# lijiaman/egoego_release

Hardware: AMD Instinct MI355X
Metric: diffusion-steps/sec (B=256, T=120, 22-joint) (higher is better)
Workload: dtype i8x3 + bf16x3 (attention layer, fc, FFN and linear_out: 2 x int8 slices per operand, int32 accumulate; embed: split-bf16, fp32 accumulate)

## Files before the change

### egoego_release_amd/csrc/egoego_hip.hip

```cpp
#include "../../include/egoego_hip.h"

#include <math.h>
#include <stdarg.h>
#include <stdio.h>
#include <stdlib.h>
#include <string.h>

#include <string>
#include <vector>

#include "attention.h"
#include "attn_layer_i8.h"
#include "attn_layer_i8w.h"
#include "attn_layer_i8h.h"
#include "attn_split_i8.h"
#include "attn_core_i8.h"
#include "attn_core_i8w.h"
#include "common.h"
#include "gemm.h"
#include "pointwise.h"
#include "tail_fused.h"

template __global__ void qkv_i8_kernel<EpiQK<2>, EpiV<2>>(QkvI8Args, EpiQK<2>, EpiV<2>);

// ... 403 lines not shown
        once.done();
    }
    if (rows / 64 >= 256) {
        c->last_kernel[EGOEGO_K_FC_LN] = FFN8 ? "tail_kernel<2,true,false>" : "tail_kernel<2,false,false>";
        tail_kernel<2, FFN8, false><<<dim3(rows / 64), dim3(256), tail_smem_bytes(2), s>>>(ta);
    } else if (!FFN8 && TAIL8_BF16 && rows / 32 <= TAIL8_BF16_MAX_BLOCKS) {
        c->last_kernel[EGOEGO_K_FC_LN] = "tail_kernel<1,false,false,false,8>";
        tail_kernel<1, false, false, false, 8><<<dim3(rows / 32), dim3(512), tail_smem_bytes(1, 8), s>>>(ta);
    } else {
        c->last_kernel[EGOEGO_K_FC_LN] = FFN8 ? "tail_kernel<1,true,false>" : "tail_kernel<1,false,false>";
        tail_kernel<1, FFN8, false><<<dim3(rows / 32), dim3(256), tail_smem_bytes(1), s>>>(ta);
    }
    HIP_TRY(hipGetLastError());
    return 0;
}
#ifndef ATTN_SPLIT_MAX_BLOCKS
#define ATTN_SPLIT_MAX_BLOCKS 256
#endif
#ifndef ATTN_SPLIT6_MAX_BLOCKS
#define ATTN_SPLIT6_MAX_BLOCKS 256
#endif
#ifndef ATTN_SPLIT2_MAX_BLOCKS
#define ATTN_SPLIT2_MAX_BLOCKS 192
#endif
#ifndef ATTN_HALF_MAX_BLOCKS
#define ATTN_HALF_MAX_BLOCKS 192
#endif
#ifndef EMBED8_MAX_BLOCKS
#define EMBED8_MAX_BLOCKS 256
#endif
#ifndef TAIL8_MAX_BLOCKS
#define TAIL8_MAX_BLOCKS 256
#endif
static int launch_tail(egoego_ctx* c, const TailArgs& ta, int rows, hipStream_t s, bool resident = false) {
    if (ta.fc8) {
        static DevOnce once;
        if (once.pending()) {
            HIP_TRY(allow_smem((tail_kernel<1, true, true, true>), tail_smem_bytes(1) + TAIL_PAR_BYTES));
            HIP_TRY(allow_smem((tail_kernel<1, true, true, false, 8>), tail_smem_bytes(1, 8) + TAIL_PAR_BYTES));
            HIP_TRY(allow_smem((tail_kernel<1, true, true, true, 4, true>), tail_smem_bytes(1) + TAIL_PAR_BYTES + TAIL_RES_BYTES));
            HIP_TRY(allow_smem((tail_kernel<1, true, true, false, 8, true>), tail_smem_bytes(1, 8) + TAIL_PAR_BYTES + TAIL_RES_BYTES));
            once.done();
        }
        if (resident) {
            if (rows / 32 > TAIL8_MAX_BLOCKS) {
                c->last_kernel[EGOEGO_K_FC_LN] = "tail_kernel<1,true,true,true,4,true>";
                tail_kernel<1, true, true, true, 4, true><<<dim3(rows / 32), dim3(256), tail_smem_bytes(1) + TAIL_PAR_BYTES + TAIL_RES_BYTES, s>>>(ta);
            } else {
                c->last_kernel[EGOEGO_K_FC_LN] = "tail_kernel<1,true,true,false,8,true>";
                tail_kernel<1, true, true, false, 8, true><<<dim3(rows / 32), dim3(512), tail_smem_bytes(1, 8) + TAIL_PAR_BYTES + TAIL_RES_BYTES, s>>>(ta);
            }
            HIP_TRY(hipGetLastError());
            return 0;
        }
        if (rows / 32 > TAIL8_MAX_BLOCKS) {
            c->last_kernel[EGOEGO_K_FC_LN] = "tail_kernel<1,true,true,true>";
            tail_kernel<1, true, true, true><<<dim3(rows / 32), dim3(256), tail_smem_bytes(1) + TAIL_PAR_BYTES, s>>>(ta);
        } else {
            c->last_kernel[EGOEGO_K_FC_LN] = "tail_kernel<1,true,true,false,8>";
            tail_kernel<1, true, true, false, 8><<<dim3(rows / 32), dim3(512), tail_smem_bytes(1, 8) + TAIL_PAR_BYTES, s>>>(ta);
        }
        HIP_TRY(hipGetLastError());
        return 0;
    }
    return ta.ffn8 ? launch_tail_f<true>(c, ta, rows, s) : launch_tail_f<false>(c, ta, rows, s);
}


template <int TT>
static int launch_embed_tt(const EmbedArgs& ea, int rows, hipStream_t s) {
    static DevOnce once;
    if (once.pending()) {
        HIP_TRY(allow_smem((embed_kernel<TT, 4>), TT * 32 * 1024));
        HIP_TRY(allow_smem((embed_kernel<TT, 8>), TT * 32 * 1024));
        once.done();
    }
    if (rows / (32 * TT) <= EMBED8_MAX_BLOCKS)
        embed_kernel<TT, 8><<<dim3(rows / (32 * TT)), dim3(512), TT * 32 * 1024, s>>>(ea);
    else
        embed_kernel<TT, 4><<<dim3(rows / (32 * TT)), dim3(256), TT * 32 * 1024, s>>>(ea);
    HIP_TRY(hipGetLastError());
    return 0;
}
template <int TT, bool I8, bool IDS>
static int launch_out_tt(const OutArgsT<IDS>& oa, int rows, hipStream_t s) {
    static DevOnce once;
    if (once.pending()) {
        HIP_TRY(allow_smem((out_kernel<TT, 1, I8, IDS>), TT * 32 * 1024));
        HIP_TRY(allow_smem((out_kernel<TT, 2, I8, IDS>), TT * 32 * 1024));
        once.done();
    }
    const int nb = rows / (32 * TT);
    if (nb <= 128)
// ... 1163 lines not shown
```

### egoego_release_amd/csrc/gemm.h

```cpp
#pragma once
#include <type_traits>

#include "common.h"

#ifndef EGOEGO_ABLATE_MAINLOOP
#define EGOEGO_ABLATE_MAINLOOP 0
#endif
#ifdef EGOEGO_PERFDEBUG
#define EG_DBG(...) __VA_ARGS__
#else
#define EG_DBG(...)
#endif

struct GemmOperands {
    const __bf16* w;
    size_t w_plane;
    const __bf16* a;
    size_t a_plane;
    int K16;
    int nfb;
    int ntb;
    int tblk0;
    EG_DBG(int ablate;
           unsigned long long* trace;)
// ... 690 lines not shown
        }
    }
};

template <int NP, int NWF, int BT>
struct EpiResLN {
    static_assert(NWF == 4 || NWF == 8, "4 waves of 4 feature tiles or 8 waves of 2");
    static EG_D float combine(const float* red, int slot) {
        float q[4];
#pragma unroll
        for (int w = 0; w < 4; ++w) q[w] = NWF == 4 ? red[slot + w * BT] : red[slot + 2 * w * BT] + red[slot + (2 * w + 1) * BT];
        return ((q[0] + q[1]) + q[2]) + q[3];
    }
    const float* bias;
    const __bf16* res;
    size_t res_plane;
    const float* gamma;
    const float* beta;
    const float* row_mask;
    __bf16* out;
    size_t out_plane;
    float eps;
    int8_t* q8;
    size_t q8_plane;
    float* q8_scale;
    const int8_t* res8;
    size_t res8_plane;
    const float* res8_scale;
    char* lds_q8;
    float* lds_scale;
    unsigned* outlier;
    float* outlier_park;
    int outlier_rows;
    template <int FT, int TT, class ResR = NoRows, class KeepR = NoRows>
    __device__ void run(f32x16 (&acc)[FT][TT], int f0, int t0, int lane, int wf, int wt, char* smem, const ResR* rr = nullptr,
                        KeepR* keep = nullptr) const {
        constexpr bool RES_REG = !std::is_same<ResR, NoRows>::value, KEEP = !std::is_same<KeepR, NoRows>::value;
        static_assert((!RES_REG && !KEEP) || TT == 1, "register rows: one token tile");
        static_assert(NWF * FT * 32 == 512 && (FT == 2 || FT == 4), "LayerNorm epilogue needs the whole 512-wide row in the block");
        const int hf = lane >> 5, col = lane & 31;
        float* red1 = (float*)smem;
        float* red2 = red1 + TT * NWF * BT;
        float* red3 = red2 + TT * NWF * BT;
        int slot[TT];
        float mean[TT], rstd[TT], amax[TT];
#pragma unroll
        for (int j = 0; j < TT; ++j) {
            const int m = t0 + j * 32 + col;
            slot[j] = (j * NWF) * BT + (wt * TT + j) * 32 + col;
            float s1 = 0.f, pp[FT / 2];
            if (RES_REG || res8) {
                float rs;
                if constexpr (RES_REG) rs = rr->scale; else rs = res8_scale[m];
#pragma unroll
                for (int i = 0; i < FT; ++i) {
                    float r[16];
                    if constexpr (RES_REG) {
                        dequant16(rr->s1[i], rr->s2[i], rs, r);
                    } else {
                        const size_t idx8 = acc_slot_i8(m, f0 + i * 32, hf, 16);
                        dequant16(*(const u32x4*)(res8 + idx8), *(const u32x4*)(res8 + res8_plane + idx8), rs, r);
                    }
#pragma unroll
                    for (int g = 0; g < 4; ++g) {
                        const float4 b4 = *(const float4*)(bias + f0 + i * 32 + 8 * g + 4 * hf);
                        const float bb[4] = {b4.x, b4.y, b4.z, b4.w};
#pragma unroll
                        for (int c = 0; c < 4; ++c) acc[i][j][4 * g + c] += bb[c] + r[4 * g + c];
                    }
                }
            } else
#pragma unroll
            for (int i = 0; i < FT; ++i)
#pragma unroll
                for (int jj = 0; jj < 2; ++jj) {
                    const int fb = f0 + i * 32 + 16 * jj + 4 * hf;
                    const float4 b0 = *(const float4*)(bias + fb);
                    const float4 b1 = *(const float4*)(bias + fb + 8);
                    const size_t idx = acc_slot(m, f0 + i * 32, jj, hf, 32);
                    float r[8];
                    const u32x4 rh = *(const u32x4*)(res + idx);
                    if (NP == 2) {
                        const u32x4 rl = *(const u32x4*)(res + res_plane + idx);
                        unpack8(rh, rl, r);
                    } else {
                        unpack8_hi(rh, r);
                    }
                    const float bb[8] = {b0.x, b0.y, b0.z, b0.w, b1.x, b1.y, b1.z, b1.w};
#pragma unroll
                    for (int c = 0; c < 8; ++c) acc[i][j][8 * jj + c] += bb[c] + r[c];
                }
#pragma unroll
            for (int i2 = 0; i2 < FT / 2; ++i2) {
                float p = 0.f;
#pragma unroll
                for (int i = 2 * i2; i < 2 * i2 + 2; ++i)
#pragma unroll
                    for (int r = 0; r < 16; ++r) p += acc[i][j][r];
                pp[i2] = p + __shfl_xor(p, 32);
            }
            s1 = pp[0];
            if (FT == 4) s1 += pp[FT / 2 - 1];
            if (hf == 0) red1[slot[j] + wf * BT] = s1;
        }
        __syncthreads();
#pragma unroll
        for (int j = 0; j < TT; ++j) {
            mean[j] = combine(red1, slot[j]) * (1.0f / 512.0f);
            float pp[FT / 2];
#pragma unroll
            for (int i2 = 0; i2 < FT / 2; ++i2) {
                float p = 0.f;
#pragma unroll
                for (int i = 2 * i2; i < 2 * i2 + 2; ++i)
#pragma unroll
                    for (int r = 0; r < 16; ++r) {
                        const float d = acc[i][j][r] - mean[j];
                        p += d * d;
                    }
                pp[i2] = p + __shfl_xor(p, 32);
            }
            float s2 = pp[0];
            if (FT == 4) s2 += pp[FT / 2 - 1];
            if (hf == 0) red2[slot[j] + wf * BT] = s2;
        }
        __syncthreads();
#pragma unroll
        for (int j = 0; j < TT; ++j) {
            const int m = t0 + j * 32 + col;
            const float var = combine(red2, slot[j]);
            rstd[j] = 1.0f / sqrtf(var * (1.0f / 512.0f) + eps);
            const float mk = row_mask ? row_mask[m] : 1.0f;
            amax[j] = 0.f;
#pragma unroll
            for (int i = 0; i < FT; ++i)
#pragma unroll
                for (int jj = 0; jj < 2; ++jj) {
                    const int fb = f0 + i * 32 + 16 * jj + 4 * hf;
                    const float4 g0 = *(const float4*)(gamma + fb), g1 = *(const float4*)(gamma + fb + 8);
                    const float4 e0 = *(const float4*)(beta + fb), e1 = *(const float4*)(beta + fb + 8);
                    const float ga[8] = {g0.x, g0.y, g0.z, g0.w, g1.x, g1.y, g1.z, g1.w};
                    const float be[8] = {e0.x, e0.y, e0.z, e0.w, e1.x, e1.y, e1.z, e1.w};
                    float v[8];
#pragma unroll
                    for (int c = 0; c < 8; ++c) {
                        v[c] = ((acc[i][j][8 * jj + c] - mean[j]) * rstd[j] * ga[c] + be[c]) * mk;
                        acc[i][j][8 * jj + c] = v[c];
                        amax[j] = fmaxf(amax[j], fabsf(v[c]));
                    }
                    if (out) {
                        u32x4 hi, lo;
                        split8(v, hi, lo);
                        const size_t idx = acc_slot(m, f0 + i * 32, jj, hf, 32);
                        *(u32x4*)(out + idx) = hi;
                        if (NP == 2) *(u32x4*)(out + out_plane + idx) = lo;
                    }
                }
            if (q8 || lds_q8) {
                amax[j] = fmaxf(amax[j], __shfl_xor(amax[j], 32));
                if (hf == 0) red3[slot[j] + wf * BT] = amax[j];
            }
        }
        if (q8 || lds_q8) {
            __syncthreads();
#pragma unroll
            for (int j = 0; j < TT; ++j) {
                const int m = t0 + j * 32 + col;
                float rmax = 0.f;
#pragma unroll
                for (int w = 0; w < NWF; ++w) rmax = fmaxf(rmax, red3[slot[j] + w * BT]);
                const float inv = rmax > 0.f ? I8_QMAX / rmax : 0.f;
                const float sc = rmax > 0.f ? rmax / I8_QMAX : 0.f;
                if (wf == 0 && hf == 0) {
                    if (q8_scale) q8_scale[m] = sc;
                    if (lds_scale) lds_scale[(wt * TT + j) * 32 + col] = sc;
                }
                if constexpr (KEEP) keep->scale = sc;
#pragma unroll
                for (int i = 0; i < FT; ++i) {
                    float v[16];
#pragma unroll
                    for (int r = 0; r < 16; ++r) v[r] = acc[i][j][r];
                    u32x4 s1, s2;
                    quant16(v, inv, s1, s2);
                    if (q8) {
                        const size_t idx = acc_slot_i8(m, f0 + i * 32, hf, 16);
                        *(u32x4*)(q8 + idx) = s1;
                        *(u32x4*)(q8 + q8_plane + idx) = s2;
                    }
                    if (lds_q8) {
                        char* d = lds_chunk_slot<TT>(lds_q8, (f0 >> 5) + i, j, lane);
                        *(u32x4*)d = s1;
                        *(u32x4*)(d + TT * 8192) = s2;
                    }
                    if constexpr (KEEP) {
                        keep->s1[i] = s1;
                        keep->s2[i] = s2;
// ... 338 lines not shown
```

### egoego_release_amd/csrc/tail_fused.h

```cpp
#pragma once
#include <type_traits>

#include "gemm.h"

#ifndef TAIL_ABLATE
#define TAIL_ABLATE 0
#endif
#ifndef TAIL_RING1
#define TAIL_RING1 4
#endif
#ifndef TAIL_RING_IO
#define TAIL_RING_IO 4
#endif
#ifndef TAIL8_RING
#define TAIL8_RING 4
#endif
#ifndef TAIL8_RING_FC
#define TAIL8_RING_FC 4
#endif

struct TailArgs {
    const __bf16* o;
    size_t o_plane;
    int HD16;
    const __bf16* wfc;
    size_t wfc_plane;
    EpiResLN<2, 4, 0> ln1;
    const __bf16* w1;
    size_t w1_plane;
    EpiTiled<true, 2> relu;
    const __bf16* w2;
    size_t w2_plane;
    EpiResLN<2, 4, 0> ln2;
    int fc8, H;
    const int8_t* o8;
    size_t o8_plane;
    const float* o_scale;
    const int8_t* wfc8;
    size_t wfc8_plane;
    const float* s_wfc;
    const int8_t* wfc8_3;
    int ffn8;
    const int8_t* w1_8;
    const int8_t* w2_8;
    size_t w8_plane;
    const float* s_w1;
    const float* s_w2;
    EpiReluQ8<4, 0> relu8;
    int stop;
    unsigned* outlier;
    int outlier_rows;
    EG_DBG(unsigned long long* trace;)
};

static constexpr int tail_smem_bytes(int TT, int NWV = 4) { return TT * 32 * 1024 + 3 * TT * NWV * 32 * TT * 4; }
static constexpr int TAIL_PAR_BYTES = 10 * 512 * 4;

using tail_rsrc = __amdgpu_buffer_rsrc_t;
EG_D tail_rsrc tail_make_rsrc(const void* p, size_t bytes) {
    return __builtin_amdgcn_make_buffer_rsrc((void*)p, 0, (int)(bytes < 0x7fffffffu ? bytes : 0x7fffffffu), 0x00020000);
}
EG_D i32x4 tail_load(tail_rsrc r, int voff, unsigned soff) {
    return __builtin_bit_cast(i32x4, __builtin_amdgcn_raw_buffer_load_b128(r, voff, soff, 0));
}

template <int FT, int TT, int RING, bool LAST, int DP, int NKS = 8, bool I8 = false, bool WLO0 = false>
struct TailChunk {
    using AccT = typename std::conditional<I8, I8Acc, f32x16>::type;
    static constexpr int PD = RING - 1, NW = FT * 2;
    static constexpr int NWL = WLO0 ? FT : NW;
    static_assert(!WLO0 || I8, "int8 slices only");
    static_assert(NKS == 8 || (LAST && DP == 0), "only the last chunk may be short");
    static_assert(RING == 2 || RING == 4 || RING == 8, "ring slots must divide the 8 k-steps of a chunk");
    static constexpr int n_ops(int s) { return ((s + PD < NKS || !LAST) ? NWL : 0) + (s == 0 ? DP : 0); }
    static constexpr int after_dma() {
        int n = 0;
        for (int s = 1; s < 8; ++s) n += n_ops(s);
        return n < 63 ? n : 63;
    }
    static constexpr int allowed(int ks) {
        int n = 0;
        if (ks < PD) {
            n += (PD - 1 - ks) * NWL;
            for (int s = 0; s < ks; ++s) n += n_ops(s);
        } else {
            n += ks - PD == 0 ? DP : 0;
            for (int s = ks - PD + 1; s < ks; ++s) n += n_ops(s);
        }
        return n < 63 ? n : 63;
    }
    template <int G>
    static EG_D void mma(i32x4 w, i32x4 a, f32x16& c) {
        if (TAIL_ABLATE & 8) return;
        c = __builtin_amdgcn_mfma_f32_32x32x16_bf16(__builtin_bit_cast(bf16x8, w), __builtin_bit_cast(bf16x8, a), c, 0, 0, 0);
    }
    template <int G>
// ... 66 lines not shown
        }
        step<0>(acc, wq, ah, al, wr, wcur, wnext, act, act_plane, lane, dma);
        if (NKS > 1) step<1>(acc, wq, ah, al, wr, wcur, wnext, act, act_plane, lane, dma);
        if (NKS > 2) step<2>(acc, wq, ah, al, wr, wcur, wnext, act, act_plane, lane, dma);
        if (NKS > 3) step<3>(acc, wq, ah, al, wr, wcur, wnext, act, act_plane, lane, dma);
        if (NKS > 4) step<4>(acc, wq, ah, al, wr, wcur, wnext, act, act_plane, lane, dma);
        if (NKS > 5) step<5>(acc, wq, ah, al, wr, wcur, wnext, act, act_plane, lane, dma);
        if (NKS > 6) step<6>(acc, wq, ah, al, wr, wcur, wnext, act, act_plane, lane, dma);
        if (NKS > 7) step<7>(acc, wq, ah, al, wr, wcur, wnext, act, act_plane, lane, dma);
        if (DP) {
            asm volatile("" ::: "memory");
            wait_counts<after_dma(), 15>();
        }
    }
};

template <int FT, int TT, int RING, bool REM2 = false, bool I8 = false, int NWAVES = 4, bool WLO0 = false>
struct DirectGemm {
    using AccT = typename std::conditional<I8, I8Acc, f32x16>::type;
    static constexpr int NW = 2 * FT, PD = RING - 1;
    static constexpr int CH_PLANE = TT * 8 * 1024, CH_BYTES = 2 * CH_PLANE;
    static constexpr int DMA_PIECES = 16 * TT / NWAVES;
    static constexpr int SMEM_BYTES = 2 * CH_BYTES;

    struct NoPost {
        EG_D void operator()(int) const {}
    };
    struct NoPre {
        EG_D void operator()() const {}
    };
    template <class Mark, class Post = NoPost, class Pre = NoPre>
    static EG_D void run(AccT (&acc)[FT][TT], const __bf16* in, size_t in_plane, int K16, const __bf16* w, size_t w_plane, char* act,
                         int tt0, int wave, int lane, Mark mark, int wtile0 = -1, Post post = Post{}, Pre pre = Pre{}) {
        const int wt0 = wtile0 >= 0 ? wtile0 : wave * FT;
        i32x4 wq[RING][NW];
        const tail_rsrc wr = tail_make_rsrc(w, w_plane * 4);
        const tail_rsrc ir = tail_make_rsrc((const char*)in + (((size_t)tt0 * (size_t)K16) << 10), 0x7fffffffu);
        const unsigned wpb = (unsigned)(w_plane * 2), ipb = (unsigned)(in_plane * 2);
        const int NQ = REM2 ? K16 / 8 + 1 : K16 / 8;
        auto w_offsets = [&](int kb, unsigned (&out)[NW]) {
#pragma unroll
            for (int i = 0; i < FT; ++i)
#pragma unroll
                for (int s = 0; s < 2; ++s) out[2 * i + s] = s * wpb + (unsigned)(((wt0 + i) * K16 + kb) << 10);
        };
        auto dma_piece = [&](int q, int piece) {
            const int x = wave * DMA_PIECES + piece;
            const int s = x / (8 * TT), j = (x >> 3) % TT;
            int kb = x & 7;
            if (REM2 && q == NQ - 1) kb &= 1;
            const unsigned src = s * ipb + (unsigned)((j * K16 + 8 * q + kb) << 10);
            char* dst = act + (q & 1) * CH_BYTES + s * CH_PLANE + ((j * 8 + kb) << 10);
            __builtin_amdgcn_raw_ptr_buffer_load_lds(ir, (__attribute__((address_space(3))) void*)dst, 16, lane * 16, src, 0, 0);
        };
        unsigned wcur[NW], wnext[NW];
#pragma unroll
        for (int pc = 0; pc < DMA_PIECES; ++pc) dma_piece(0, pc);
        w_offsets(0, wcur);
#pragma unroll
        for (int k = 0; k < PD; ++k)
#pragma unroll
            for (int q = 0; q < NW; ++q)
                if (!(WLO0 && (q & 1))) wq[k][q] = tail_load(wr, lane * 16, wcur[q] + (k << 10));
#pragma unroll
        for (int i = 0; i < FT; ++i)
#pragma unroll
            for (int j = 0; j < TT; ++j) acc_zero(acc[i][j]);
        pre();
        asm volatile("s_waitcnt vmcnt(0)" ::: "memory");
        __syncthreads();
        mark();
        for (int q = 0; q + 1 < NQ; ++q) {
            w_offsets(8 * q, wcur);
            w_offsets(8 * q + 8, wnext);
            TailChunk<FT, TT, RING, false, DMA_PIECES, 8, I8, WLO0>::run(acc, wq, wr, wcur, wnext, act + (q & 1) * CH_BYTES, CH_PLANE, lane,
                                                             [&](int piece) { dma_piece(q + 1, piece); });
            post(q);
            __builtin_amdgcn_s_barrier();
            asm volatile("" ::: "memory");
        }
        w_offsets(8 * (NQ - 1), wcur);
        TailChunk<FT, TT, RING, true, 0, (REM2 ? 2 : 8), I8, WLO0>::run(acc, wq, wr, wcur, wcur, act + ((NQ - 1) & 1) * CH_BYTES, CH_PLANE, lane, [](int) {});
        post(NQ - 1);
        __syncthreads();
    }

    static EG_D void prime(i32x4 (&wq)[RING][NW], const __bf16* w, size_t w_plane, int K16, int wt0, int lane) {
        const tail_rsrc wr = tail_make_rsrc(w, w_plane * 4);
        const unsigned wpb = (unsigned)(w_plane * 2);
#pragma unroll
        for (int k = 0; k < PD; ++k)
#pragma unroll
            for (int i = 0; i < FT; ++i)
#pragma unroll
                for (int sl = 0; sl < 2; ++sl) wq[k][2 * i + sl] = tail_load(wr, lane * 16, sl * wpb + (unsigned)(((wt0 + i) * K16 + k) << 10));
    }
    template <class Mark>
    static EG_D void run_resident(AccT (&acc)[FT][TT], i32x4 (&wq)[RING][NW], const __bf16* w, size_t w_plane, const char* act, int lane, Mark mark,
                                  int wt0) {
        static_assert(!REM2, "two whole chunks");
        constexpr int K16 = 16;
        const tail_rsrc wr = tail_make_rsrc(w, w_plane * 4);
        const unsigned wpb = (unsigned)(w_plane * 2);
        auto w_offsets = [&](int kb, unsigned (&out)[NW]) {
#pragma unroll
            for (int i = 0; i < FT; ++i)
#pragma unroll
                for (int sl = 0; sl < 2; ++sl) out[2 * i + sl] = sl * wpb + (unsigned)(((wt0 + i) * K16 + kb) << 10);
        };
        unsigned wcur[NW], wnext[NW];
#pragma unroll
        for (int i = 0; i < FT; ++i)
#pragma unroll
            for (int j = 0; j < TT; ++j) acc_zero(acc[i][j]);
        mark();
        w_offsets(0, wcur);
        w_offsets(8, wnext);
        TailChunk<FT, TT, RING, false, 0, 8, I8>::run(acc, wq, wr, wcur, wnext, act, CH_PLANE, lane, [](int) {});
        TailChunk<FT, TT, RING, true, 0, 8, I8>::run(acc, wq, wr, wnext, wnext, act + CH_BYTES, CH_PLANE, lane, [](int) {});
    }
};

static constexpr int TAIL_RES_BYTES = 272;
template <int TT, bool FFN8, bool FC8 = false, bool W2 = false, int NWV = 4, bool RES = false>
__global__ __launch_bounds__(64 * NWV, ((W2 || NWV == 8) ? 2 : 1)) void tail_kernel(TailArgs a) {
    static_assert(!RES || (FFN8 && FC8 && TT == 1), "LDS-resident FFN operands: the all-int8 32-token tail");
    static_assert(!W2 || (FFN8 && FC8 && TT == 1), "the two-workgroups-per-CU build exists for the all-int8 32-token tail");
    static_assert(NWV == 4 || (NWV == 8 && TT == 1 && !W2 && ((FFN8 && FC8) || (!FFN8 && !FC8 && !RES))),
                  "the eight-wave build exists for the 32-token tails: all int8, or (round 5) all split-bf16");
    constexpr int TOK = 32 * TT, FT = 16 / NWV;
    using G = DirectGemm<FT, TT, 4, false, false, NWV>;
    extern __shared__ __attribute__((aligned(16))) char smem[];
    char* const act = smem;
    char* const red = smem + G::SMEM_BYTES;
    const int wave = wave_id_uniform();
    const int lane = threadIdx.x & 63;
    const int tok0 = (int)blockIdx.x * TOK;
    const int tt0 = (int)blockIdx.x * TT;
    EG_DBG(unsigned long long* const tr = a.trace ? a.trace + 180224 + (size_t)blockIdx.x * 32 : nullptr;)
    auto mark = [&](int i) {
        EG_DBG(if (tr && threadIdx.x == 0) {
            tr[i] = wall_clock64();
            tr[16 + i] = __builtin_readcyclecounter();
        })
        (void)i;
    };
    mark(0);
    f32x16 acc[FT][TT];
    auto as_ln = [&](const EpiResLN<2, 4, 0>& e, int which = 0) {
        return EpiResLN<2, NWV, TOK>{e.bias, e.res, e.res_plane, e.gamma, e.beta, e.row_mask, e.out, e.out_plane, e.eps, e.q8, e.q8_plane, e.q8_scale, e.res8, e.res8_plane, e.res8_scale, nullptr, nullptr,
                                     a.outlier ? a.outlier + which : nullptr, nullptr, a.outlier_rows};
    };
    const float *p_swfc = a.s_wfc, *p_sw1 = a.s_w1, *p_sw2 = a.s_w2;
    const float* const par_src[10] = {a.s_wfc, a.ln1.bias, a.ln1.gamma, a.ln1.beta, a.s_w1, a.relu8.bias, a.s_w2, a.ln2.bias, a.ln2.gamma, a.ln2.beta};
    auto stage_params = [&] {
        float* par = (float*)(smem + tail_smem_bytes(TT, NWV));
        if (threadIdx.x < 128) {
#pragma unroll
            for (int v = 0; v < 10; ++v) *(float4*)(par + v * 512 + 4 * threadIdx.x) = *(const float4*)(par_src[v] + 4 * threadIdx.x);
        }
    };
    if constexpr (FFN8 && FC8) {
        float* par = (float*)(smem + tail_smem_bytes(TT, NWV));
        p_swfc = par;
        a.ln1.bias = par + 512; a.ln1.gamma = par + 1024; a.ln1.beta = par + 1536;
        p_sw1 = par + 2048; a.relu8.bias = par + 2560;
        p_sw2 = par + 3072; a.ln2.bias = par + 3584; a.ln2.gamma = par + 4096; a.ln2.beta = par + 4608;
    }

    if constexpr (FC8) {
        constexpr int FP = NWV == 8 ? 1 : ((W2 || TAIL_RING1 == 8) ? 2 : TT), FTP = FT / FP;
        using GF = DirectGemm<FTP, TT, (NWV == 8 ? TAIL8_RING_FC : (W2 ? 4 : TAIL_RING1)), false, true, NWV>;
        const int col = lane & 31;
#pragma unroll
        for (int i = 0; i < FT; ++i)
#pragma unroll
            for (int j = 0; j < TT; ++j)
#pragma unroll
                for (int r = 0; r < 16; ++r) acc[i][j][r] = 0.f;
#pragma unroll
        for (int fp = 0; fp < FP; ++fp) {
            I8Acc q[FTP][TT];
            GF::run(q, (const __bf16*)a.o8, a.o8_plane / 2, a.HD16 / 2, (const __bf16*)a.wfc8, a.wfc8_plane / 2, act, tt0, wave, lane, [&] { mark(7); },
                    wave * FT + fp * FTP, [&](int h) {
                        float so[TT];
#pragma unroll
                        for (int j = 0; j < TT; ++j) so[j] = a.o_scale[(size_t)(tok0 + j * 32 + col) * a.H + h] * 256.0f;
#pragma unroll
                        for (int i = 0; i < FTP; ++i)
#pragma unroll
                            for (int j = 0; j < TT; ++j) {
                                i8_fold(q[i][j], acc[fp * FTP + i][j], so[j]);
                                acc_zero(q[i][j]);
                            }
                    }, [&] { if (fp == 0) stage_params(); });
        }
        if (a.wfc8_3) {
#pragma unroll
            for (int fp = 0; fp < FP; ++fp) {
                I8Acc q[FTP][TT];
                using GF3 = DirectGemm<FTP, TT, (NWV == 8 ? TAIL8_RING_FC : (W2 ? 4 : TAIL_RING1)), false, true, NWV, true>;
                GF3::run(q, (const __bf16*)a.o8, a.o8_plane / 2, a.HD16 / 2, (const __bf16*)a.wfc8_3, a.wfc8_plane / 2, act, tt0, wave, lane, [&] {},
                        wave * FT + fp * FTP, [&](int h) {
                            float so[TT];
#pragma unroll
                            for (int j = 0; j < TT; ++j) so[j] = a.o_scale[(size_t)(tok0 + j * 32 + col) * a.H + h] * (1.0f / 256.0f);
#pragma unroll
                            for (int i = 0; i < FTP; ++i)
#pragma unroll
                                for (int j = 0; j < TT; ++j) {
                                    i8_fold(q[i][j], acc[fp * FTP + i][j], so[j]);
                                    acc_zero(q[i][j]);
                                }
                        });
            }
        }
#pragma unroll
        for (int i = 0; i < FT; ++i)
#pragma unroll
            for (int j = 0; j < TT; ++j) i8_fold_finish(acc[i][j], p_swfc + wave * FT * 32 + i * 32 + 4 * (lane >> 5));
    } else {
        G::run(acc, a.o, a.o_plane, a.HD16, a.wfc, a.wfc_plane, act, tt0, wave, lane, [&] { mark(7); });
    }
    mark(1);
    if constexpr (RES) {
        constexpr int FP8 = W2 ? 2 : 1, FTP8 = FT / FP8, RING8 = NWV == 8 ? TAIL8_RING : 4;
        using G8 = DirectGemm<FTP8, TT, RING8, false, true, NWV>;
        float* const ls1 = (float*)(smem + tail_smem_bytes(TT, NWV) + TAIL_PAR_BYTES);
        float* const ls2 = ls1 + 32;
        i32x4 wq[RING8][2 * FTP8];
        Rows8<FT> h1;
        auto ffn_resident = [&](I8Acc (&q)[FT][TT], const int8_t* w8, int mk) {
#pragma unroll
            for (int fp = 0; fp < FP8; ++fp) {
                if (fp) G8::prime(wq, (const __bf16*)w8, a.w8_plane / 2, 16, wave * FT + fp * FTP8, lane);
                G8::run_resident(*(I8Acc(*)[FTP8][TT]) & q[fp * FTP8], wq, (const __bf16*)w8, a.w8_plane / 2, act, lane, [&] { mark(mk); }, wave * FT + fp * FTP8);
            }
        };
        G8::prime(wq, (const __bf16*)a.w1_8, a.w8_plane / 2, 16, wave * FT, lane);
        {
            auto e = as_ln(a.ln1);
            if (a.stop != 1) { e.q8 = nullptr; e.q8_scale = nullptr; }
            e.lds_q8 = act; e.lds_scale = ls1;
            if (e.outlier) { e.outlier = nullptr; e.outlier_park = ls2 + 32; }
            e.template run<FT, TT, NoRows, Rows8<FT>>(acc, wave * FT * 32, tok0, lane, wave, 0, red, nullptr, &h1);
        }
        if (a.stop == 1) return;
        __syncthreads();
        mark(2);
        I8Acc q[FT][TT];
        ffn_resident(q, a.w1_8, 8);
        mark(3);
        G8::prime(wq, (const __bf16*)a.w2_8, a.w8_plane / 2, 16, wave * FT, lane);
        {
            const bool tap = a.stop == 2;
            const EpiReluQ8<NWV, TOK> e{a.relu8.bias, tap ? a.relu8.q8 : nullptr, a.relu8.q8_plane, tap ? a.relu8.q8_scale : nullptr, act, ls2, tap ? tok0 : 0};
            e.template run<false, I8Acc, FT, TT>(q, p_sw1, ls1, wave * FT * 32, 0, lane, wave, 0, red);
        }
        if (a.stop == 2) return;
        __syncthreads();
        mark(4);
        ffn_resident(q, a.w2_8, 9);
        mark(5);
        i8_dequant_tile<false>(q, acc, p_sw2, ls2, wave * FT * 32, 0, lane);
        {
            auto e = as_ln(a.ln2, 1);
            e.res8 = nullptr;
            e.template run<FT, TT, Rows8<FT>, NoRows>(acc, wave * FT * 32, tok0, lane, wave, 0, red, &h1, nullptr);
        }
        if (a.outlier && threadIdx.x == 0) atomicMax(a.outlier, __builtin_bit_cast(unsigned, ls2[32]));
        EG_DBG(if (tr) { asm volatile("s_waitcnt vmcnt(0)" ::: "memory"); })
        mark(6);
        return;
    }
    as_ln(a.ln1).template run<FT, TT>(acc, wave * FT * 32, tok0, lane, wave, 0, red);
    asm volatile("s_waitcnt vmcnt(0)" ::: "memory");
    __syncthreads();
    mark(2);
    if (a.stop == 1) return;

    if constexpr (FFN8) {
        constexpr int FP8 = NWV == 8 ? 1 : ((W2 || (TT == 1 && TAIL_RING1 == 8)) ? 2 : 1), FTP8 = FT / FP8;
        using G8 = DirectGemm<FTP8, TT, (TT == 2 ? 2 : (W2 ? 4 : (NWV == 8 ? TAIL8_RING : TAIL_RING1))), false, true, NWV>;
        const EpiReluQ8<NWV, TOK> e8{a.relu8.bias, a.relu8.q8, a.relu8.q8_plane, a.relu8.q8_scale};
        auto ffn_gemm = [&](I8Acc (&q)[FT][TT], const int8_t* in8, size_t in_plane_bytes, const int8_t* w8, int mk) {
#pragma unroll
            for (int fp = 0; fp < FP8; ++fp)
                G8::run(*(I8Acc(*)[FTP8][TT]) & q[fp * FTP8], (const __bf16*)in8, in_plane_bytes / 2, 16, (const __bf16*)w8, a.w8_plane / 2, act, tt0, wave,
                        lane, [&] { mark(mk); }, wave * FT + fp * FTP8);
        };
        {
            I8Acc q[FT][TT];
            ffn_gemm(q, a.ln1.q8, a.ln1.q8_plane, a.w1_8, 8);
            mark(3);
            e8.template run<false, I8Acc, FT, TT>(q, p_sw1, a.ln1.q8_scale, wave * FT * 32, tok0, lane, wave, 0, red);
        }
        asm volatile("s_waitcnt vmcnt(0)" ::: "memory");
        __syncthreads();
        mark(4);
        if (a.stop == 2) return;
        {
            I8Acc q[FT][TT];
            ffn_gemm(q, a.relu8.q8, a.relu8.q8_plane, a.w2_8, 9);
            mark(5);
            i8_dequant_tile<false>(q, acc, p_sw2, a.relu8.q8_scale, wave * FT * 32, tok0, lane);
        }
        as_ln(a.ln2, 1).template run<FT, TT>(acc, wave * FT * 32, tok0, lane, wave, 0, red);
        EG_DBG(if (tr) { asm volatile("s_waitcnt vmcnt(0)" ::: "memory"); })
        mark(6);
        return;
    }
    if constexpr (!FFN8) {
    G::run(acc, a.ln1.out, a.ln1.out_plane, 32, a.w1, a.w1_plane, act, tt0, wave, lane, [&] { mark(8); });
    mark(3);
    a.relu.template run<FT, TT>(acc, wave * FT * 32, tok0, lane, wave, 0, red);
    asm volatile("s_waitcnt vmcnt(0)" ::: "memory");
    __syncthreads();
    mark(4);
    if (a.stop == 2) return;

    G::run(acc, a.relu.out, a.relu.out_plane, 32, a.w2, a.w2_plane, act, tt0, wave, lane, [&] { mark(9); });
    mark(5);
    as_ln(a.ln2, 1).template run<FT, TT>(acc, wave * FT * 32, tok0, lane, wave, 0, red);
    EG_DBG(if (tr) { asm volatile("s_waitcnt vmcnt(0)" ::: "memory"); })
    mark(6);
    }
}

struct EmbedArgs {
    const __bf16* x;
    size_t x_plane;
    int K16;
    const __bf16* w;
    size_t w_plane;
    EpiEmbed<2, 4, 0> epi;
};
template <int TT, int NWV = 4>
__global__ __launch_bounds__(64 * NWV, (NWV == 8 ? 2 : 1)) void embed_kernel(EmbedArgs a) {
    constexpr int FT = 16 / NWV;
    using G = DirectGemm<FT, TT, TAIL_RING_IO, true, false, NWV>;
    extern __shared__ __attribute__((aligned(16))) char smem[];
    const int wave = wave_id_uniform(), lane = threadIdx.x & 63;
    f32x16 acc[FT][TT];
    G::run(acc, a.x, a.x_plane, a.K16, a.w, a.w_plane, smem, (int)blockIdx.x * TT, wave, lane, [] {});
    const EpiEmbed<2, NWV, 32 * TT> e{a.epi.bias, a.epi.pe, a.epi.tt_table, a.epi.t_idx, a.epi.out, a.epi.out_plane, a.epi.Lp, a.epi.T, a.epi.B,
                                      a.epi.q8, a.epi.q8_plane, a.epi.q8_scale, a.epi.state, a.epi.ts};
    e.template run<FT, TT>(acc, wave * FT * 32, (int)blockIdx.x * 32 * TT, lane, wave, 0, smem);
}

template <bool IDS = false>
struct OutArgsT {
    const __bf16* h;
    size_t h_plane;
    const __bf16* w;
    size_t w_plane;
    EpiOut<2, IDS> epi;
    const int8_t* h8;
    size_t h8_plane;
// ... 28 lines not shown
```

Baseline: 771.9.

## Make resident int8 tail kernel persistent with cross-tile prefetch and LDS-staged scalars

The resident int8 tail kernel becomes a persistent grid of about two workgroups per CU that walks the token tiles. During the final LayerNorm of one tile it prefetches the next tile's first activation chunk and its per-head/residual scales into LDS, and it primes the fc weights before each tile. Per-token o_scale and res8_scale reads now come from double-buffered LDS instead of global memory, and some LayerNorm barriers become lighter s_barrier waits. The aim is to hide launch and prologue latency between tiles. The cost is more LDS use, inline-asm DMA that the compiler cannot track, and a new n_head limit.

```diff
diff --git a/egoego_release_amd/csrc/egoego_hip.hip b/egoego_release_amd/csrc/egoego_hip.hip
--- a/egoego_release_amd/csrc/egoego_hip.hip
+++ b/egoego_release_amd/csrc/egoego_hip.hip
@@ -459,33 +459,43 @@
 #ifndef TAIL8_MAX_BLOCKS
 #define TAIL8_MAX_BLOCKS 256
 #endif
-static int launch_tail(egoego_ctx* c, const TailArgs& ta, int rows, hipStream_t s, bool resident = false) {
+static int launch_tail(egoego_ctx* c, const TailArgs& ta_in, int rows, hipStream_t s, bool resident = false) {
+    TailArgs ta = ta_in;
+    ta.nblocks = rows / 32;
     if (ta.fc8) {
+        constexpr int smem4 = tail_smem_bytes(1) + TAIL_PAR_BYTES + TAIL_SC_BYTES, smem8 = tail_smem_bytes(1, 8) + TAIL_PAR_BYTES + TAIL_SC_BYTES;
+        static_assert(2 * (smem4 + TAIL_RES_BYTES) <= 160 * 1024, "two four-wave workgroups per CU");
         static DevOnce once;
+        static int n_cu[64];
         if (once.pending()) {
-            HIP_TRY(allow_smem((tail_kernel<1, true, true, true>), tail_smem_bytes(1) + TAIL_PAR_BYTES));
-            HIP_TRY(allow_smem((tail_kernel<1, true, true, false, 8>), tail_smem_bytes(1, 8) + TAIL_PAR_BYTES));
-            HIP_TRY(allow_smem((tail_kernel<1, true, true, true, 4, true>), tail_smem_bytes(1) + TAIL_PAR_BYTES + TAIL_RES_BYTES));
-            HIP_TRY(allow_smem((tail_kernel<1, true, true, false, 8, true>), tail_smem_bytes(1, 8) + TAIL_PAR_BYTES + TAIL_RES_BYTES));
+            HIP_TRY(allow_smem((tail_kernel<1, true, true, true>), smem4));
+            HIP_TRY(allow_smem((tail_kernel<1, true, true, false, 8>), smem8));
+            HIP_TRY(allow_smem((tail_kernel<1, true, true, true, 4, true>), smem4 + TAIL_RES_BYTES));
+            HIP_TRY(allow_smem((tail_kernel<1, true, true, false, 8, true>), smem8 + TAIL_RES_BYTES));
+            int cu = 0;
+            HIP_TRY(hipDeviceGetAttribute(&cu, hipDeviceAttributeMultiprocessorCount, once.dev));
+            n_cu[once.dev & 63] = cu;
             once.done();
         }
+        if (ta.H > TAIL_SC_MAXH) return fail(EGOEGO_E_INVALID, "n_head=%d: the tail stages at most %d heads' scales", ta.H, TAIL_SC_MAXH);
         if (resident) {
             if (rows / 32 > TAIL8_MAX_BLOCKS) {
+                const int grid = TAIL_WALK ? std::min(rows / 32, 2 * std::max(1, n_cu[once.dev & 63])) : rows / 32;
                 c->last_kernel[EGOEGO_K_FC_LN] = "tail_kernel<1,true,true,true,4,true>";
-                tail_kernel<1, true, true, true, 4, true><<<dim3(rows / 32), dim3(256), tail_smem_bytes(1) + TAIL_PAR_BYTES + TAIL_RES_BYTES, s>>>(ta);
+                tail_kernel<1, true, true, true, 4, true><<<dim3(grid), dim3(256), smem4 + TAIL_RES_BYTES, s>>>(ta);
             } else {
                 c->last_kernel[EGOEGO_K_FC_LN] = "tail_kernel<1,true,true,false,8,true>";
-                tail_kernel<1, true, true, false, 8, true><<<dim3(rows / 32), dim3(512), tail_smem_bytes(1, 8) + TAIL_PAR_BYTES + TAIL_RES_BYTES, s>>>(ta);
+                tail_kernel<1, true, true, false, 8, true><<<dim3(rows / 32), dim3(512), smem8 + TAIL_RES_BYTES, s>>>(ta);
             }
             HIP_TRY(hipGetLastError());
             return 0;
         }
         if (rows / 32 > TAIL8_MAX_BLOCKS) {
             c->last_kernel[EGOEGO_K_FC_LN] = "tail_kernel<1,true,true,true>";
-            tail_kernel<1, true, true, true><<<dim3(rows / 32), dim3(256), tail_smem_bytes(1) + TAIL_PAR_BYTES, s>>>(ta);
+            tail_kernel<1, true, true, true><<<dim3(rows / 32), dim3(256), smem4, s>>>(ta);
         } else {
             c->last_kernel[EGOEGO_K_FC_LN] = "tail_kernel<1,true,true,false,8>";
-            tail_kernel<1, true, true, false, 8><<<dim3(rows / 32), dim3(512), tail_smem_bytes(1, 8) + TAIL_PAR_BYTES, s>>>(ta);
+            tail_kernel<1, true, true, false, 8><<<dim3(rows / 32), dim3(512), smem8, s>>>(ta);
         }
         HIP_TRY(hipGetLastError());
         return 0;
diff --git a/egoego_release_amd/csrc/gemm.h b/egoego_release_amd/csrc/gemm.h
--- a/egoego_release_amd/csrc/gemm.h
+++ b/egoego_release_amd/csrc/gemm.h
@@ -746,10 +746,26 @@
     unsigned* outlier;
     float* outlier_park;
     int outlier_rows;
-    template <int FT, int TT, class ResR = NoRows, class KeepR = NoRows>
+    const float* lds_res8_scale;
+    struct NoHook {
+        EG_D void operator()() const {}
+    };
+    template <bool LIGHT>
+    static EG_D void exchange_barrier() {
+        if constexpr (LIGHT) {
+            asm volatile("" ::: "memory");
+            wait_counts<63, 0>();
+            __builtin_amdgcn_s_barrier();
+            asm volatile("" ::: "memory");
+        } else {
+            __syncthreads();
+        }
+    }
+    template <int FT, int TT, class ResR = NoRows, class KeepR = NoRows, class Hook = NoHook>
     __device__ void run(f32x16 (&acc)[FT][TT], int f0, int t0, int lane, int wf, int wt, char* smem, const ResR* rr = nullptr,
-                        KeepR* keep = nullptr) const {
+                        KeepR* keep = nullptr, Hook hook = Hook{}) const {
         constexpr bool RES_REG = !std::is_same<ResR, NoRows>::value, KEEP = !std::is_same<KeepR, NoRows>::value;
+        constexpr bool LIGHT = !std::is_same<Hook, NoHook>::value;
         static_assert((!RES_REG && !KEEP) || TT == 1, "register rows: one token tile");
         static_assert(NWF * FT * 32 == 512 && (FT == 2 || FT == 4), "LayerNorm epilogue needs the whole 512-wide row in the block");
         const int hf = lane >> 5, col = lane & 31;
@@ -758,6 +774,11 @@
         float* red3 = red2 + TT * NWF * BT;
         int slot[TT];
         float mean[TT], rstd[TT], amax[TT];
+        [[maybe_unused]] float mk_early[TT];
+        if constexpr (LIGHT) {
+#pragma unroll
+            for (int j = 0; j < TT; ++j) mk_early[j] = row_mask ? row_mask[t0 + j * 32 + col] : 1.0f;
+        }
 #pragma unroll
         for (int j = 0; j < TT; ++j) {
             const int m = t0 + j * 32 + col;
@@ -765,7 +786,7 @@
             float s1 = 0.f, pp[FT / 2];
             if (RES_REG || res8) {
                 float rs;
-                if constexpr (RES_REG) rs = rr->scale; else rs = res8_scale[m];
+                if constexpr (RES_REG) rs = rr->scale; else rs = lds_res8_scale ? lds_res8_scale[(wt * TT + j) * 32 + col] : res8_scale[m];
 #pragma unroll
                 for (int i = 0; i < FT; ++i) {
                     float r[16];
@@ -818,6 +839,11 @@
             if (hf == 0) red1[slot[j] + wf * BT] = s1;
         }
         __syncthreads();
+        if constexpr (LIGHT) {
+#pragma unroll
+            for (int j = 0; j < TT; ++j) asm volatile("" ::"v"(mk_early[j]));
+        }
+        hook();
 #pragma unroll
         for (int j = 0; j < TT; ++j) {
             mean[j] = combine(red1, slot[j]) * (1.0f / 512.0f);
@@ -838,13 +864,14 @@
             if (FT == 4) s2 += pp[FT / 2 - 1];
             if (hf == 0) red2[slot[j] + wf * BT] = s2;
         }
-        __syncthreads();
+        exchange_barrier<LIGHT>();
 #pragma unroll
         for (int j = 0; j < TT; ++j) {
             const int m = t0 + j * 32 + col;
             const float var = combine(red2, slot[j]);
             rstd[j] = 1.0f / sqrtf(var * (1.0f / 512.0f) + eps);
-            const float mk = row_mask ? row_mask[m] : 1.0f;
+            float mk;
+            if constexpr (LIGHT) mk = mk_early[j]; else mk = row_mask ? row_mask[m] : 1.0f;
             amax[j] = 0.f;
 #pragma unroll
             for (int i = 0; i < FT; ++i)
@@ -876,7 +903,7 @@
             }
         }
         if (q8 || lds_q8) {
-            __syncthreads();
+            exchange_barrier<LIGHT>();
 #pragma unroll
             for (int j = 0; j < TT; ++j) {
                 const int m = t0 + j * 32 + col;
diff --git a/egoego_release_amd/csrc/tail_fused.h b/egoego_release_amd/csrc/tail_fused.h
--- a/egoego_release_amd/csrc/tail_fused.h
+++ b/egoego_release_amd/csrc/tail_fused.h
@@ -17,6 +17,13 @@
 #endif
 #ifndef TAIL8_RING_FC
 #define TAIL8_RING_FC 4
+#endif
+
+#ifndef TAIL_LDS_SCALARS
+#define TAIL_LDS_SCALARS 1
+#endif
+#ifndef TAIL_WALK
+#define TAIL_WALK 1
 #endif
 
 struct TailArgs {
@@ -50,11 +57,15 @@
     int stop;
     unsigned* outlier;
     int outlier_rows;
+    int nblocks;
     EG_DBG(unsigned long long* trace;)
 };
 
 static constexpr int tail_smem_bytes(int TT, int NWV = 4) { return TT * 32 * 1024 + 3 * TT * NWV * 32 * TT * 4; }
 static constexpr int TAIL_PAR_BYTES = 10 * 512 * 4;
+static constexpr int TAIL_SC_MAXH = 16;
+static constexpr int TAIL_SC_BUF = 32 * TAIL_SC_MAXH * 4 + 256;
+static constexpr int TAIL_SC_BYTES = 2 * TAIL_SC_BUF;
 
 using tail_rsrc = __amdgpu_buffer_rsrc_t;
 EG_D tail_rsrc tail_make_rsrc(const void* p, size_t bytes) {
@@ -62,6 +73,21 @@
 }
 EG_D i32x4 tail_load(tail_rsrc r, int voff, unsigned soff) {
     return __builtin_bit_cast(i32x4, __builtin_amdgcn_raw_buffer_load_b128(r, voff, soff, 0));
+}
+
+template <int BYTES>
+EG_D void tail_dma_unseen(const void* base, unsigned bytes, void* lds, int voff, unsigned soff) {
+    static_assert(BYTES == 4 || BYTES == 16, "dword or dwordx4");
+    const unsigned long long b = (unsigned long long)base;
+    const i32x4 r = {(int)(unsigned)b, (int)((unsigned)(b >> 32) & 0xffffu), (int)(bytes < 0x7fffffffu ? bytes : 0x7fffffffu), 0x00020000};
+    const unsigned dst = (unsigned)(unsigned long long)(__attribute__((address_space(3))) char*)lds;
+    unsigned keep;
+    if constexpr (BYTES == 16)
+        asm volatile("s_nop 4\n\ts_mov_b32 %0, m0\n\ts_mov_b32 m0, %1\n\ts_nop 0\n\tbuffer_load_dwordx4 %2, %3, %4 offen lds\n\ts_mov_b32 m0, %0"
+                     : "=&s"(keep) : "s"(dst), "v"(voff), "s"(r), "s"(soff) : "memory");
+    else
+        asm volatile("s_nop 4\n\ts_mov_b32 %0, m0\n\ts_mov_b32 m0, %1\n\ts_nop 0\n\tbuffer_load_dword %2, %3, %4 offen lds\n\ts_mov_b32 m0, %0"
+                     : "=&s"(keep) : "s"(dst), "v"(voff), "s"(r), "s"(soff) : "memory");
 }
 
 template <int FT, int TT, int RING, bool LAST, int DP, int NKS = 8, bool I8 = false, bool WLO0 = false>
@@ -194,8 +220,28 @@
     template <class Mark, class Post = NoPost, class Pre = NoPre>
     static EG_D void run(AccT (&acc)[FT][TT], const __bf16* in, size_t in_plane, int K16, const __bf16* w, size_t w_plane, char* act,
                          int tt0, int wave, int lane, Mark mark, int wtile0 = -1, Post post = Post{}, Pre pre = Pre{}) {
+        i32x4 wq[RING][NW];
+        run_ring<false>(acc, wq, in, in_plane, K16, w, w_plane, act, tt0, wave, lane, mark, wtile0, post, pre);
+    }
+    template <bool UNSEEN = false>
+    static EG_D void request_first_chunk(const __bf16* in, size_t in_plane, int K16, char* act, int tt0, int wave, int lane) {
+        static_assert(!REM2, "whole chunks");
+        const char* const base = (const char*)in + (((size_t)tt0 * (size_t)K16) << 10);
+        const tail_rsrc ir = tail_make_rsrc(base, 0x7fffffffu);
+        const unsigned ipb = (unsigned)(in_plane * 2);
+#pragma unroll
+        for (int pc = 0; pc < DMA_PIECES; ++pc) {
+            const int x = wave * DMA_PIECES + pc, s = x / (8 * TT), j = (x >> 3) % TT, kb = x & 7;
+            char* const dst = act + s * CH_PLANE + ((j * 8 + kb) << 10);
+            const unsigned src = s * ipb + (unsigned)((j * K16 + kb) << 10);
+            if constexpr (UNSEEN) tail_dma_unseen<16>(base, 0x7fffffffu, dst, lane * 16, src);
+            else __builtin_amdgcn_raw_ptr_buffer_load_lds(ir, (__attribute__((address_space(3))) void*)dst, 16, lane * 16, src, 0, 0);
+        }
+    }
+    template <bool PRIMED, class Mark, class Post = NoPost, class Pre = NoPre>
+    static EG_D void run_ring(AccT (&acc)[FT][TT], i32x4 (&wq)[RING][NW], const __bf16* in, size_t in_plane, int K16, const __bf16* w, size_t w_plane,
+                              char* act, int tt0, int wave, int lane, Mark mark, int wtile0 = -1, Post post = Post{}, Pre pre = Pre{}) {
         const int wt0 = wtile0 >= 0 ? wtile0 : wave * FT;
-        i32x4 wq[RING][NW];
         const tail_rsrc wr = tail_make_rsrc(w, w_plane * 4);
         const tail_rsrc ir = tail_make_rsrc((const char*)in + (((size_t)tt0 * (size_t)K16) << 10), 0x7fffffffu);
         const unsigned wpb = (unsigned)(w_plane * 2), ipb = (unsigned)(in_plane * 2);
@@ -216,21 +262,31 @@
             __builtin_amdgcn_raw_ptr_buffer_load_lds(ir, (__attribute__((address_space(3))) void*)dst, 16, lane * 16, src, 0, 0);
         };
         unsigned wcur[NW], wnext[NW];
-#pragma unroll
-        for (int pc = 0; pc < DMA_PIECES; ++pc) dma_piece(0, pc);
-        w_offsets(0, wcur);
-#pragma unroll
-        for (int k = 0; k < PD; ++k)
-#pragma unroll
-            for (int q = 0; q < NW; ++q)
-                if (!(WLO0 && (q & 1))) wq[k][q] = tail_load(wr, lane * 16, wcur[q] + (k << 10));
+        if constexpr (!PRIMED) {
+#pragma unroll
+            for (int pc = 0; pc < DMA_PIECES; ++pc) dma_piece(0, pc);
+            w_offsets(0, wcur);
+#pragma unroll
+            for (int k = 0; k < PD; ++k)
+#pragma unroll
+                for (int q = 0; q < NW; ++q)
+                    if (!(WLO0 && (q & 1))) wq[k][q] = tail_load(wr, lane * 16, wcur[q] + (k << 10));
+        }
 #pragma unroll
         for (int i = 0; i < FT; ++i)
 #pragma unroll
             for (int j = 0; j < TT; ++j) acc_zero(acc[i][j]);
-        pre();
-        asm volatile("s_waitcnt vmcnt(0)" ::: "memory");
-        __syncthreads();
+        if constexpr (PRIMED) {
+            static_assert(!WLO0 && PD * NW <= 63, "prime() loads both slices");
+            asm volatile("" ::: "memory");
+            wait_counts<PD * NW, 0>();
+            __builtin_amdgcn_s_barrier();
+            asm volatile("" ::: "memory");
+        } else {
+            pre();
+            asm volatile("s_waitcnt vmcnt(0)" ::: "memory");
+            __syncthreads();
+        }
         mark();
         for (int q = 0; q + 1 < NQ; ++q) {
             w_offsets(8 * q, wcur);
@@ -285,21 +341,25 @@
 
 static constexpr int TAIL_RES_BYTES = 272;
 template <int TT, bool FFN8, bool FC8 = false, bool W2 = false, int NWV = 4, bool RES = false>
-__global__ __launch_bounds__(64 * NWV, ((W2 || NWV == 8) ? 2 : 1)) void tail_kernel(TailArgs a) {
+__global__ __launch_bounds__(64 * NWV, ((W2 || NWV == 8) ? 2 : 1)) void tail_kernel(TailArgs a_in) {
     static_assert(!RES || (FFN8 && FC8 && TT == 1), "LDS-resident FFN operands: the all-int8 32-token tail");
     static_assert(!W2 || (FFN8 && FC8 && TT == 1), "the two-workgroups-per-CU build exists for the all-int8 32-token tail");
     static_assert(NWV == 4 || (NWV == 8 && TT == 1 && !W2 && ((FFN8 && FC8) || (!FFN8 && !FC8 && !RES))),
                   "the eight-wave build exists for the 32-token tails: all int8, or (round 5) all split-bf16");
     constexpr int TOK = 32 * TT, FT = 16 / NWV;
     using G = DirectGemm<FT, TT, 4, false, false, NWV>;
+    TailArgs a = a_in;
+    constexpr bool WALK = TAIL_WALK && W2 && RES;
+    constexpr bool SC = TAIL_LDS_SCALARS && FC8;
+    constexpr int FP = NWV == 8 ? 1 : ((W2 || TAIL_RING1 == 8) ? 2 : TT), FTP = FT / FP;
+    using GF = DirectGemm<FTP, TT, (NWV == 8 ? TAIL8_RING_FC : (W2 ? 4 : TAIL_RING1)), false, true, NWV>;
     extern __shared__ __attribute__((aligned(16))) char smem[];
     char* const act = smem;
     char* const red = smem + G::SMEM_BYTES;
-    const int wave = wave_id_uniform();
-    const int lane = threadIdx.x & 63;
-    const int tok0 = (int)blockIdx.x * TOK;
-    const int tt0 = (int)blockIdx.x * TT;
-    EG_DBG(unsigned long long* const tr = a.trace ? a.trace + 180224 + (size_t)blockIdx.x * 32 : nullptr;)
+    char* const sc_area = smem + tail_smem_bytes(TT, NWV) + TAIL_PAR_BYTES + (RES ? TAIL_RES_BYTES : 0);
+    int wave = wave_id_uniform();
+    int lane = threadIdx.x & 63;
+    EG_DBG(unsigned long long* tr = nullptr;)
     auto mark = [&](int i) {
         EG_DBG(if (tr && threadIdx.x == 0) {
             tr[i] = wall_clock64();
@@ -307,33 +367,80 @@
         })
         (void)i;
     };
-    mark(0);
+    auto stage_scalars = [&](int t0, char* buf, auto unseen) {
+        if (wave != 0) return;
+        const float* const so = a.o_scale + (size_t)t0 * a.H;
+        const unsigned so_bytes = (unsigned)(TOK * a.H * 4);
+        const tail_rsrc r = tail_make_rsrc(so, so_bytes);
+        for (int i = 0; i < (TOK * a.H * 4 + 255) / 256; ++i) {
+            if constexpr (unseen.value) tail_dma_unseen<4>(so, so_bytes, buf + i * 256, lane * 4, i * 256);
+            else __builtin_amdgcn_raw_ptr_buffer_load_lds(r, (__attribute__((address_space(3))) void*)(buf + i * 256), 4, lane * 4, i * 256, 0, 0);
+        }
+        if (a.ln1.res8) {
+            const tail_rsrc r8 = tail_make_rsrc(a.ln1.res8_scale + t0, (size_t)TOK * 4);
+            char* const dst = buf + TOK * TAIL_SC_MAXH * 4;
+            if constexpr (unseen.value) tail_dma_unseen<4>(a.ln1.res8_scale + t0, TOK * 4, dst, lane * 4, 0);
+            else __builtin_amdgcn_raw_ptr_buffer_load_lds(r8, (__attribute__((address_space(3))) void*)dst, 4, lane * 4, 0, 0, 0);
+        }
+    };
+    static_assert(!SC || TT == 1, "TAIL_SC_BUF holds one token tile's scalars");
     f32x16 acc[FT][TT];
     auto as_ln = [&](const EpiResLN<2, 4, 0>& e, int which = 0) {
         return EpiResLN<2, NWV, TOK>{e.bias, e.res, e.res_plane, e.gamma, e.beta, e.row_mask, e.out, e.out_plane, e.eps, e.q8, e.q8_plane, e.q8_scale, e.res8, e.res8_plane, e.res8_scale, nullptr, nullptr,
-                                     a.outlier ? a.outlier + which : nullptr, nullptr, a.outlier_rows};
+                                     a.outlier ? a.outlier + which : nullptr, nullptr, a.outlier_rows, nullptr};
     };
     const float *p_swfc = a.s_wfc, *p_sw1 = a.s_w1, *p_sw2 = a.s_w2;
-    const float* const par_src[10] = {a.s_wfc, a.ln1.bias, a.ln1.gamma, a.ln1.beta, a.s_w1, a.relu8.bias, a.s_w2, a.ln2.bias, a.ln2.gamma, a.ln2.beta};
     auto stage_params = [&] {
+        const TailArgs& o = a_in;
+        const float* const par_src[10] = {o.s_wfc, o.ln1.bias, o.ln1.gamma, o.ln1.beta, o.s_w1, o.relu8.bias, o.s_w2, o.ln2.bias, o.ln2.gamma, o.ln2.beta};
         float* par = (float*)(smem + tail_smem_bytes(TT, NWV));
-        if (threadIdx.x < 128) {
-#pragma unroll
-            for (int v = 0; v < 10; ++v) *(float4*)(par + v * 512 + 4 * threadIdx.x) = *(const float4*)(par_src[v] + 4 * threadIdx.x);
-        }
-    };
-    if constexpr (FFN8 && FC8) {
-        float* par = (float*)(smem + tail_smem_bytes(TT, NWV));
-        p_swfc = par;
-        a.ln1.bias = par + 512; a.ln1.gamma = par + 1024; a.ln1.beta = par + 1536;
-        p_sw1 = par + 2048; a.relu8.bias = par + 2560;
-        p_sw2 = par + 3072; a.ln2.bias = par + 3584; a.ln2.gamma = par + 4096; a.ln2.beta = par + 4608;
+        const int tid = WALK ? wave * 64 + lane : (int)threadIdx.x;
+        if (tid < 128) {
+#pragma unroll
+            for (int v = 0; v < 10; ++v) *(float4*)(par + v * 512 + 4 * tid) = *(const float4*)(par_src[v] + 4 * tid);
+        }
+    };
+    auto use_lds_params = [&] {
+        if constexpr (FFN8 && FC8) {
+            float* par = (float*)(smem + tail_smem_bytes(TT, NWV));
+            p_swfc = par;
+            a.ln1.bias = par + 512; a.ln1.gamma = par + 1024; a.ln1.beta = par + 1536;
+            p_sw1 = par + 2048; a.relu8.bias = par + 2560;
+            p_sw2 = par + 3072; a.ln2.bias = par + 3584; a.ln2.gamma = par + 4096; a.ln2.beta = par + 4608;
+        }
+    };
+    use_lds_params();
+
+    const int nblk = WALK ? a.nblocks : (int)blockIdx.x + 1;
+    [[maybe_unused]] bool requested = false;
+    for (int blk = (int)blockIdx.x, it = 0; blk < nblk; blk += (int)gridDim.x, ++it) {
+    if constexpr (WALK) {
+        asm volatile("" : "+v"(lane));
+        asm volatile("" : "+s"(wave));
+        wave = __builtin_amdgcn_readfirstlane(wave);
+    }
+    const int tok0 = blk * TOK;
+    const int tt0 = blk * TT;
+    EG_DBG(tr = a.trace ? a.trace + 180224 + (size_t)blk * 32 : nullptr;)
+    mark(0);
+    char* const scb = sc_area + (it & 1) * TAIL_SC_BUF;
+    const float* const so_lds = (const float*)scb;
+    const float* const rs_lds = (const float*)(scb + TOK * TAIL_SC_MAXH * 4);
+    auto o_scale_of = [&](int j, int h) {
+        const int col = lane & 31;
+        return SC ? so_lds[(j * 32 + col) * a.H + h] : a.o_scale[(size_t)(tok0 + j * 32 + col) * a.H + h];
+    };
+    [[maybe_unused]] i32x4 wqf[WALK ? 4 : 1][2 * FTP];
+    if constexpr (WALK) {
+        if (!requested) {
+            GF::request_first_chunk((const __bf16*)a.o8, a.o8_plane / 2, a.HD16 / 2, act, tt0, wave, lane);
+            if (SC) stage_scalars(tok0, scb, std::false_type{});
+        }
+        GF::prime(wqf, (const __bf16*)a.wfc8, a.wfc8_plane / 2, a.HD16 / 2, wave * FT, lane);
+        if (it == 0) stage_params();
     }
 
     if constexpr (FC8) {
-        constexpr int FP = NWV == 8 ? 1 : ((W2 || TAIL_RING1 == 8) ? 2 : TT), FTP = FT / FP;
-        using GF = DirectGemm<FTP, TT, (NWV == 8 ? TAIL8_RING_FC : (W2 ? 4 : TAIL_RING1)), false, true, NWV>;
-        const int col = lane & 31;
 #pragma unroll
         for (int i = 0; i < FT; ++i)
 #pragma unroll
@@ -343,19 +450,31 @@
 #pragma unroll
         for (int fp = 0; fp < FP; ++fp) {
             I8Acc q[FTP][TT];
-            GF::run(q, (const __bf16*)a.o8, a.o8_plane / 2, a.HD16 / 2, (const __bf16*)a.wfc8, a.wfc8_plane / 2, act, tt0, wave, lane, [&] { mark(7); },
-                    wave * FT + fp * FTP, [&](int h) {
-                        float so[TT];
-#pragma unroll
-                        for (int j = 0; j < TT; ++j) so[j] = a.o_scale[(size_t)(tok0 + j * 32 + col) * a.H + h] * 256.0f;
-#pragma unroll
-                        for (int i = 0; i < FTP; ++i)
-#pragma unroll
-                            for (int j = 0; j < TT; ++j) {
-                                i8_fold(q[i][j], acc[fp * FTP + i][j], so[j]);
-                                acc_zero(q[i][j]);
+            auto fold = [&](int h) {
+                float so[TT];
+#pragma unroll
+                for (int j = 0; j < TT; ++j) so[j] = o_scale_of(j, h) * 256.0f;
+#pragma unroll
+                for (int i = 0; i < FTP; ++i)
+#pragma unroll
+                    for (int j = 0; j < TT; ++j) {
+                        i8_fold(q[i][j], acc[fp * FTP + i][j], so[j]);
+                        acc_zero(q[i][j]);
+                    }
+            };
+            if (WALK && fp == 0) {
+                if constexpr (WALK)
+                    GF::template run_ring<true>(q, wqf, (const __bf16*)a.o8, a.o8_plane / 2, a.HD16 / 2, (const __bf16*)a.wfc8, a.wfc8_plane / 2, act, tt0, wave, lane,
+                                                [&] { mark(7); }, wave * FT, fold);
+            } else {
+                GF::run(q, (const __bf16*)a.o8, a.o8_plane / 2, a.HD16 / 2, (const __bf16*)a.wfc8, a.wfc8_plane / 2, act, tt0, wave, lane, [&] { mark(7); },
+                        wave * FT + fp * FTP, fold, [&] {
+                            if (fp == 0) {
+                                if (SC) stage_scalars(tok0, scb, std::false_type{});
+                                stage_params();
                             }
-                    }, [&] { if (fp == 0) stage_params(); });
+                        });
+            }
         }
         if (a.wfc8_3) {
 #pragma unroll
@@ -366,7 +485,7 @@
                         wave * FT + fp * FTP, [&](int h) {
                             float so[TT];
 #pragma unroll
-                            for (int j = 0; j < TT; ++j) so[j] = a.o_scale[(size_t)(tok0 + j * 32 + col) * a.H + h] * (1.0f / 256.0f);
+                            for (int j = 0; j < TT; ++j) so[j] = o_scale_of(j, h) * (1.0f / 256.0f);
 #pragma unroll
                             for (int i = 0; i < FTP; ++i)
 #pragma unroll
@@ -392,6 +511,7 @@
         float* const ls2 = ls1 + 32;
         i32x4 wq[RING8][2 * FTP8];
         Rows8<FT> h1;
+        if constexpr (WALK) h1 = Rows8<FT>{};
         auto ffn_resident = [&](I8Acc (&q)[FT][TT], const int8_t* w8, int mk) {
 #pragma unroll
             for (int fp = 0; fp < FP8; ++fp) {
@@ -404,10 +524,16 @@
             auto e = as_ln(a.ln1);
             if (a.stop != 1) { e.q8 = nullptr; e.q8_scale = nullptr; }
             e.lds_q8 = act; e.lds_scale = ls1;
+            if (SC && e.res8) e.lds_res8_scale = rs_lds;
             if (e.outlier) { e.outlier = nullptr; e.outlier_park = ls2 + 32; }
             e.template run<FT, TT, NoRows, Rows8<FT>>(acc, wave * FT * 32, tok0, lane, wave, 0, red, nullptr, &h1);
         }
-        if (a.stop == 1) return;
+        if (a.stop == 1) {
+            if (!WALK) return;
+            __syncthreads();
+            requested = false;
+            continue;
+        }
         __syncthreads();
         mark(2);
         I8Acc q[FT][TT];
@@ -419,7 +545,12 @@
             const EpiReluQ8<NWV, TOK> e{a.relu8.bias, tap ? a.relu8.q8 : nullptr, a.relu8.q8_plane, tap ? a.relu8.q8_scale : nullptr, act, ls2, tap ? tok0 : 0};
             e.template run<false, I8Acc, FT, TT>(q, p_sw1, ls1, wave * FT * 32, 0, lane, wave, 0, red);
         }
-        if (a.stop == 2) return;
+        if (a.stop == 2) {
+            if (!WALK) return;
+            __syncthreads();
+            requested = false;
+            continue;
+        }
         __syncthreads();
         mark(4);
         ffn_resident(q, a.w2_8, 9);
@@ -428,14 +559,32 @@
         {
             auto e = as_ln(a.ln2, 1);
             e.res8 = nullptr;
-            e.template run<FT, TT, Rows8<FT>, NoRows>(acc, wave * FT * 32, tok0, lane, wave, 0, red, &h1, nullptr);
+            if constexpr (WALK) {
+                const int nxt = blk + (int)gridDim.x;
+                e.template run<FT, TT, Rows8<FT>, NoRows>(acc, wave * FT * 32, tok0, lane, wave, 0, red, &h1, nullptr, [&] {
+                    if (nxt < nblk) {
+                        GF::template request_first_chunk<true>((const __bf16*)a.o8, a.o8_plane / 2, a.HD16 / 2, act, nxt * TT, wave, lane);
+                        if (SC) stage_scalars(nxt * TOK, sc_area + ((it + 1) & 1) * TAIL_SC_BUF, std::true_type{});
+                    }
+                });
+            } else {
+                e.template run<FT, TT, Rows8<FT>, NoRows>(acc, wave * FT * 32, tok0, lane, wave, 0, red, &h1, nullptr);
+            }
         }
         if (a.outlier && threadIdx.x == 0) atomicMax(a.outlier, __builtin_bit_cast(unsigned, ls2[32]));
         EG_DBG(if (tr) { asm volatile("s_waitcnt vmcnt(0)" ::: "memory"); })
         mark(6);
+        if constexpr (WALK) {
+            requested = true;
+            continue;
+        }
         return;
     }
-    as_ln(a.ln1).template run<FT, TT>(acc, wave * FT * 32, tok0, lane, wave, 0, red);
+    {
+        auto e = as_ln(a.ln1);
+        if (SC && e.res8) e.lds_res8_scale = rs_lds;
+        e.template run<FT, TT>(acc, wave * FT * 32, tok0, lane, wave, 0, red);
+    }
     asm volatile("s_waitcnt vmcnt(0)" ::: "memory");
     __syncthreads();
     mark(2);
@@ -486,6 +635,8 @@
     as_ln(a.ln2, 1).template run<FT, TT>(acc, wave * FT * 32, tok0, lane, wave, 0, red);
     EG_DBG(if (tr) { asm volatile("s_waitcnt vmcnt(0)" ::: "memory"); })
     mark(6);
+    }
+    return;
     }
 }
 
```

Result: slower. 750.5 (-2.8%).
